# qdrant/quantization

Measured on AMD Instinct MI355X. Metric: scored vectors/sec, 10Mx768 u8 dot, higher is better.
Workload: dtype u8; 1 GPU; 10000000 x 768 store: f32 U[0,1) -> scalar u8 (dot); per step: encode_query + score_all over the shard; quantizer=u8, rows_per_gpu=10000000, dim=768, distance=dot, exchange=scores, gather_group=1, launch=single rank, world_size_seen=1, encode_ahead=False, total_rows=10000000, queries=16

## Files before the change

### quantization_amd/csrc/u8.hip

```cpp
#include <algorithm>
#include <cmath>
#include <cstdlib>
#include <memory>
#include <type_traits>
#include <vector>

#include "common.hpp"
#include "lists.hpp"
#include "multi_reduce.hpp"
#include "topk.hpp"
#include "topk_device.hpp"
#include "rescore.hpp"
#include "u8_internal.hpp"

#pragma clang fp contract(off)

using namespace qamd;

namespace {

constexpr int kBlock = 256;
constexpr int kScanBlock = 512;
constexpr uint64_t kQuantileSample = 100000;

enum Epilogue : int { EPI_POINT = 0, EPI_INTERNAL = 1 };

typedef uint32_t u32x4 __attribute__((ext_vector_type(4)));
typedef float f32x4 __attribute__((ext_vector_type(4)));

__device__ __forceinline__ uint4 ld_nt(const uint4 *p) {
    u32x4 t = __builtin_nontemporal_load(reinterpret_cast<const u32x4 *>(p));
    return make_uint4(t.x, t.y, t.z, t.w);
}
__device__ __forceinline__ float4 ld_nt(const float4 *p) {
    f32x4 t = __builtin_nontemporal_load(reinterpret_cast<const f32x4 *>(p));
    return make_float4(t.x, t.y, t.z, t.w);
}

__device__ __forceinline__ uint32_t dot16(const uint4 &a, const uint4 &b, uint32_t acc) {
    acc = __builtin_amdgcn_udot4(a.x, b.x, acc, false);
    acc = __builtin_amdgcn_udot4(a.y, b.y, acc, false);
    acc = __builtin_amdgcn_udot4(a.z, b.z, acc, false);
    acc = __builtin_amdgcn_udot4(a.w, b.w, acc, false);
    return acc;
}

__device__ __forceinline__ uint32_t sad16(const uint4 &a, const uint4 &b, uint32_t acc) {
    acc = __builtin_amdgcn_sad_u8(a.x, b.x, acc);
    acc = __builtin_amdgcn_sad_u8(a.y, b.y, acc);
    acc = __builtin_amdgcn_sad_u8(a.z, b.z, acc);
    acc = __builtin_amdgcn_sad_u8(a.w, b.w, acc);
    return acc;
}

template <int CTRL> __device__ __forceinline__ uint32_t dpp_add(uint32_t v) {
    return v + (uint32_t)__builtin_amdgcn_update_dpp(0, (int)v, CTRL, 0xF, 0xF, false);
}
template <int G> __device__ __forceinline__ uint32_t group_sum(uint32_t v) {
    static_assert(G == 1 || G == 2 || G == 4 || G == 8 || G == 16, "row group is at most one DPP row");
    if (G >= 2) v = dpp_add<0xB1>(v);
    if (G >= 4) v = dpp_add<0x4E>(v);
    if (G >= 8) v = dpp_add<0x141>(v);
    if (G >= 16) v = dpp_add<0x140>(v);
    return v;
}

__device__ __forceinline__ float epilogue_f(float multiplier, float sf, float q_off, float v_off, float diff, int mode) {
    float ms = multiplier * sf;
    if (mode == EPI_POINT) return (ms + q_off) + v_off;
    return ms + ((q_off + v_off) - diff);
}
__device__ __forceinline__ float epilogue(float multiplier, uint32_t s, float q_off, float v_off,
                                          float diff, int mode) {
    return epilogue_f(multiplier, (float)(int32_t)s, q_off, v_off, diff, mode);
}

__device__ __forceinline__ void dot16_lanes(const uint4 &v, const uint4 &q, uint32_t (&acc)[8]) {
    const uint32_t vd[4] = {v.x, v.y, v.z, v.w};
    const uint32_t qd[4] = {q.x, q.y, q.z, q.w};
#pragma unroll
    for (int j = 0; j < 4; j++) {
        acc[2 * j] = __builtin_amdgcn_udot4(vd[j], qd[j] & 0x0000FFFFu, acc[2 * j], false);
        acc[2 * j + 1] = __builtin_amdgcn_udot4(vd[j], qd[j] & 0xFFFF0000u, acc[2 * j + 1], false);
    }
}
template <int G> __device__ __forceinline__ float avx2_lane_sum(uint32_t (&acc)[8]) {
    float f[8];
#pragma unroll
    for (int k = 0; k < 8; k++) f[k] = (float)(int32_t)group_sum<G>(acc[k]);
    float a0 = f[0] + f[4], a1 = f[1] + f[5], a2 = f[2] + f[6], a3 = f[3] + f[7];
    return (a0 + a2) + (a1 + a3);
}

__device__ __forceinline__ uint32_t f32_to_u8(float v, float alpha, float offset) {
    float x = (v - offset) / alpha;
    x = (x < 0.0f) ? 0.0f : x;
    x = (x > 127.0f) ? 127.0f : x;
    return (x != x) ? 0u : (uint32_t)x;
}

__device__ __forceinline__ bool quant_decided(float y) {
    constexpr float kBand = 3.0517578125e-05f;
    const float fr = __builtin_amdgcn_fractf(y);
    return (__builtin_fabsf(fr - 0.5f) <= 0.5f - kBand) || (__builtin_fabsf(y - 64.0f) >= 64.0f + kBand);
}
__device__ __forceinline__ uint32_t quant_code(float y) {
    return (uint32_t)__builtin_amdgcn_fmed3f(y, 0.0f, 127.0f);
}
__device__ __forceinline__ uint32_t f32x4_to_u8x4_fast(const float4 &f, float alpha, float offset, float r_alpha) {
    const float y0 = (f.x - offset) * r_alpha, y1 = (f.y - offset) * r_alpha, y2 = (f.z - offset) * r_alpha,
                y3 = (f.w - offset) * r_alpha;
    if (quant_decided(y0) && quant_decided(y1) && quant_decided(y2) && quant_decided(y3))
        return quant_code(y0) | (quant_code(y1) << 8) | (quant_code(y2) << 16) | (quant_code(y3) << 24);
    return f32_to_u8(f.x, alpha, offset) | (f32_to_u8(f.y, alpha, offset) << 8) | (f32_to_u8(f.z, alpha, offset) << 16) |
           (f32_to_u8(f.w, alpha, offset) << 24);
}

template <int G, int ITERS, int UNROLL, bool IS_L1, bool EXACT, bool FILTER>
__global__ __launch_bounds__(kScanBlock) void u8_scan_kernel(
    const uint4 *__restrict__ codes, const float *__restrict__ offsets,
    const uint4 *__restrict__ qcodes, const float *__restrict__ q_off_p, float multiplier,
    uint32_t n_rows, uint32_t row_chunks, float *__restrict__ out, TopkFilter filt) {
    constexpr int RW = 64 / G;
    constexpr int TILE = RW * UNROLL;
    const int lane = threadIdx.x & 63;
    const int sub = lane % G;
    const int rslot = lane / G;
    const uint64_t wave = ((uint64_t)blockIdx.x * kScanBlock + threadIdx.x) >> 6;
    const uint64_t base = wave * TILE;
    if (base >= n_rows) return;

    uint4 v[UNROLL][ITERS];
#pragma unroll
    for (int u = 0; u < UNROLL; u++) {
        const uint64_t row = base + u * RW + rslot;
        const uint4 *p = codes + row * row_chunks;
#pragma unroll
        for (int it = 0; it < ITERS; it++) {
            const uint32_t c = sub + it * G;
            if (EXACT) {
                v[u][it] = ld_nt(p + c);
            } else {
                const uint32_t cc = c < row_chunks ? c : row_chunks - 1;
                uint4 t = ld_nt(p + cc);
                const bool in = c < row_chunks;
                v[u][it] = make_uint4(in ? t.x : 0, in ? t.y : 0, in ? t.z : 0, in ? t.w : 0);
            }
        }
    }
    uint4 q[ITERS];
#pragma unroll
    for (int it = 0; it < ITERS; it++) {
        const uint32_t c = sub + it * G;
        if (EXACT) {
            q[it] = qcodes[c];
        } else {
            const uint4 t = qcodes[c < row_chunks ? c : row_chunks - 1];
            const bool in = c < row_chunks;
            q[it] = make_uint4(in ? t.x : 0, in ? t.y : 0, in ? t.z : 0, in ? t.w : 0);
        }
    }
    const float q_off = *q_off_p;
    constexpr int NGROUPS = (UNROLL + G - 1) / G;
    float v_off[NGROUPS];
#pragma unroll
    for (int g = 0; g < NGROUPS; g++)
        v_off[g] = offsets[base + (uint64_t)(g * G + sub) * RW + rslot];
    float mine = 0.0f;
    uint32_t pivot = 0;
    if (FILTER) pivot = *filt.pivot_key;
#pragma unroll
    for (int u = 0; u < UNROLL; u++) {
        uint32_t acc = 0;
#pragma unroll
        for (int it = 0; it < ITERS; it++) acc = IS_L1 ? sad16(v[u][it], q[it], acc) : dot16(v[u][it], q[it], acc);
        acc = group_sum<G>(acc);
        if (sub == (u % G)) mine = epilogue(multiplier, acc, q_off, v_off[u / G], 0.0f, EPI_POINT);
        if ((u % G) == G - 1 || u == UNROLL - 1) {
            constexpr int dummy = 0;
            (void)dummy;
            const int first = (u / G) * G;
            const uint64_t row = base + (uint64_t)(first + sub) * RW + rslot;
            if (sub <= u - first && row < n_rows) {
                if (FILTER) topk_offer(filt, pivot, mine, (uint32_t)row);
                else __builtin_nontemporal_store(mine, out + row);
            }
        }
    }
}

constexpr uint32_t kPackBlockRows = 64;
constexpr uint32_t kPackBlockChunk = kPackBlockRows;

__device__ __forceinline__ uint4 and16(const uint4 &v, uint32_t m) { return make_uint4(v.x & m, v.y & m, v.z & m, v.w & m); }

template <bool FILTER>
__global__ __launch_bounds__(kScanBlock) __attribute__((amdgpu_waves_per_eu(8, 8))) void u8_scan_blocked_kernel(
    const uint4 *__restrict__ image, const float *__restrict__ offsets, const uint4 *__restrict__ qcodes,
    const float *__restrict__ q_off_p, float multiplier, uint32_t n_rows, uint32_t pchunks, uint32_t n_extra,
    uint32_t split, float *__restrict__ out, TopkFilter filt) {
    __shared__ uint32_t partial[kScanBlock];
    const uint32_t lane = threadIdx.x & 63;
    const uint32_t wave = __builtin_amdgcn_readfirstlane(threadIdx.x >> 6);
    const uint32_t part = wave & (split - 1);
    const uint64_t block = (uint64_t)blockIdx.x * ((kScanBlock / 64) / split) + wave / split;
    const uint64_t row = block * kPackBlockRows + lane;
    const bool live = block * kPackBlockRows < n_rows;
    const uint32_t n_rest = pchunks - 7 * n_extra, n_groups = n_extra + (n_rest ? 1 : 0);
    const uint32_t g_begin = live ? n_groups * part / split : 0, g_end = live ? n_groups * (part + 1) / split : 0;
    const uint4 *blk = image + block * pchunks * kPackBlockChunk;
    const uint32_t lane16 = lane * 16;
    auto chunk_ptr = [&](uint32_t c) {
        return reinterpret_cast<const uint4 *>(reinterpret_cast<const char *>(blk + (uint64_t)c * kPackBlockChunk) + lane16);
    };
    const uint32_t gf_end = g_end < n_extra ? g_end : n_extra;
    const bool has_rest = g_end > n_extra;

    uint4 v[7];
    uint32_t acc = 0;
    auto eat = [&](uint32_t g, auto refill) {
        const uint4 *q = qcodes + 7 * g;
        const uint4 qx = qcodes[pchunks + g];
#pragma unroll
        for (int i = 0; i < 7; i++) {
            const uint4 w = v[i];
            acc = dot16(and16(w, 0x7F7F7F7Fu), q[i], acc) + (dot16(and16(w, 0x80808080u), qx, 0) >> (7 - i));
            if (decltype(refill)::value) {
                __builtin_amdgcn_sched_barrier(0);
                v[i] = ld_nt(chunk_ptr(7 * (g + 1) + i));
                __builtin_amdgcn_sched_barrier(0);
            }
        }
    };
    if (g_begin < gf_end) {
#pragma unroll
        for (int i = 0; i < 7; i++) v[i] = ld_nt(chunk_ptr(7 * g_begin + i));
    }
    const float v_off = offsets[row];
    const float q_off = *q_off_p;
    uint32_t pivot = 0;
    if (FILTER) pivot = *filt.pivot_key;
    if (g_begin < gf_end) {
        for (uint32_t g = g_begin; g + 1 < gf_end; g++) eat(g, std::true_type{});
        eat(gf_end - 1, std::false_type{});
    }
    if (has_rest) {
        const uint4 *q = qcodes + 7 * n_extra;
#pragma unroll
        for (int i = 0; i < 7; i++)
            if ((uint32_t)i < n_rest) v[i] = ld_nt(chunk_ptr(7 * n_extra + i));
#pragma unroll
        for (int i = 0; i < 7; i++)
            if ((uint32_t)i < n_rest) acc = dot16(and16(v[i], 0x7F7F7F7Fu), q[i], acc);
    }
    if (split > 1) {
        partial[threadIdx.x] = acc;
        __syncthreads();
        if (part == 0)
            for (uint32_t p = 1; p < split; p++) acc += partial[threadIdx.x + 64 * p];
    }
    if (part == 0 && row < n_rows) {
        const float score = epilogue(multiplier, acc, q_off, v_off, 0.0f, EPI_POINT);
        if (FILTER) topk_offer(filt, pivot, score, (uint32_t)row);
        else __builtin_nontemporal_store(score, out + row);
    }
}

template <int G, int ITERS, int UNROLL, int NQ, bool IS_L1, bool EXACT, bool FILTER>
__global__ __launch_bounds__(kScanBlock) void u8_scan_multi_kernel(
    const uint4 *__restrict__ codes, const float *__restrict__ offsets, const uint8_t *__restrict__ qcodes,
    uint32_t q_pitch, const float *__restrict__ q_offs, uint32_t nq_valid ,
    float multiplier, uint32_t n_rows, uint32_t row_chunks, float *__restrict__ out ,
    uint64_t out_pitch, TopkFilterSlices slices) {
    static_assert(G >= NQ, "one lane of the row group per query");
    constexpr int RW = 64 / G;
    constexpr int TILE = RW * UNROLL;
    constexpr int TPW = NQ;
    const int lane = threadIdx.x & 63;
    const int sub = lane % G, rslot = lane / G;
    const uint64_t wave = ((uint64_t)blockIdx.x * kScanBlock + threadIdx.x) >> 6;
    if (wave * TILE * TPW >= n_rows) return;
    uint4 q[NQ][ITERS];
#pragma unroll
    for (int j = 0; j < NQ; j++) {
        const uint4 *qj = reinterpret_cast<const uint4 *>(qcodes + (size_t)((uint32_t)j < nq_valid ? j : nq_valid - 1) * q_pitch);
#pragma unroll
        for (int it = 0; it < ITERS; it++) {
            const uint32_t c = sub + it * G;
            const bool in = EXACT || c < row_chunks;
            const uint4 t = qj[in ? c : row_chunks - 1];
            q[j][it] = make_uint4(in ? t.x : 0, in ? t.y : 0, in ? t.z : 0, in ? t.w : 0);
        }
    }
    const int my_q = multi_query_of<NQ>(sub);
    const bool owner = sub < NQ && (uint32_t)my_q < nq_valid;
    const float q_off = q_offs[owner ? my_q : 0];
    for (int tile = 0; tile < TPW; tile++) {
        const uint64_t base = (wave * TPW + tile) * TILE;
        if (base >= n_rows) break;
        uint4 v[UNROLL][ITERS];
#pragma unroll
        for (int u = 0; u < UNROLL; u++) {
            const uint4 *p = codes + (base + u * RW + rslot) * row_chunks;
#pragma unroll
            for (int it = 0; it < ITERS; it++) {
                const uint32_t c = sub + it * G;
                const bool in = EXACT || c < row_chunks;
                const uint4 t = ld_nt(p + (in ? c : row_chunks - 1));
                v[u][it] = make_uint4(in ? t.x : 0, in ? t.y : 0, in ? t.z : 0, in ? t.w : 0);
            }
        }
#pragma unroll
        for (int u = 0; u < UNROLL; u++) {
            const uint64_t row = base + (uint64_t)u * RW + rslot;
            const float v_off = offsets[row];
            uint32_t acc[NQ];
#pragma unroll
            for (int j = 0; j < NQ; j++) {
                acc[j] = 0;
#pragma unroll
                for (int it = 0; it < ITERS; it++)
                    acc[j] = IS_L1 ? sad16(v[u][it], q[j][it], acc[j]) : dot16(v[u][it], q[j][it], acc[j]);
            }
            const float mine = epilogue(multiplier, multi_reduce<G, NQ>(acc, sub), q_off, v_off, 0.0f, EPI_POINT);
            if (owner && row < n_rows) {
                if (FILTER) {
                    const TopkFilter f = topk_filter_of(slices, (uint32_t)my_q);
                    topk_offer(f, *f.pivot_key, mine, (uint32_t)row);
                } else {
                    __builtin_nontemporal_store(mine, out + (uint64_t)my_q * out_pitch + row);
                }
            }
        }
    }
}

template <int G, int ITERS, bool IS_L1, bool EXACT>
__device__ __forceinline__ void u8_topk_small_body(const uint4 *__restrict__ codes, const float *__restrict__ offsets,
                                                   const uint4 (&q)[ITERS], float q_off, float multiplier, uint32_t n_rows,
                                                   uint32_t row_chunks, uint32_t rows_per_wg, const SmallTopk &p,
                                                   unsigned long long (*lds)[64]) {
    unsigned long long(*lists)[64] = lds;
    constexpr int RW = 64 / G;
    constexpr int UNROLL = 2;
    const int lane = threadIdx.x & 63, wave = threadIdx.x >> 6;
    const int sub = lane % G, rslot = lane / G;
    unsigned long long *stage = lds[kSmallTopkWaves + wave];
    const uint64_t wg_base = (uint64_t)blockIdx.x * rows_per_wg;
    SmallTopkWave acc_list;
    for (uint32_t tile = wave * UNROLL; tile * RW < rows_per_wg; tile += kSmallTopkWaves * UNROLL) {
        uint4 v[UNROLL][ITERS];
#pragma unroll
        for (int u = 0; u < UNROLL; u++) {
            const uint64_t row = wg_base + (uint64_t)(tile + u) * RW + rslot;
            const uint64_t rc = row < n_rows ? row : (uint64_t)n_rows - 1;
            const uint4 *src = codes + rc * row_chunks;
#pragma unroll
            for (int it = 0; it < ITERS; it++) {
// ... 587 lines not shown
        uint32_t k = (uint32_t)(t - r * row_dwords);
        uint32_t w = rows32[t];
        if (k == 0)
            offsets[r] = __uint_as_float(w);
        else
            codes32[r * (row_dwords - 1) + (k - 1)] = w;
    }
}

__global__ __launch_bounds__(kBlock) void join_rows_kernel(const uint32_t *__restrict__ codes32,
                                                          const float *__restrict__ offsets,
                                                          uint64_t n_rows, uint32_t row_dwords,
                                                          uint32_t *__restrict__ rows32) {
    const uint64_t total = n_rows * row_dwords;
    const uint64_t stride = (uint64_t)gridDim.x * kBlock;
    for (uint64_t t = (uint64_t)blockIdx.x * kBlock + threadIdx.x; t < total; t += stride) {
        uint64_t r = t / row_dwords;
        uint32_t k = (uint32_t)(t - r * row_dwords);
        rows32[t] = k == 0 ? __float_as_uint(offsets[r]) : codes32[r * (row_dwords - 1) + (k - 1)];
    }
}

__global__ __launch_bounds__(kBlock) void u8_pack7_kernel(const uint4 *__restrict__ codes, uint64_t n_rows,
                                                          uint32_t row_chunks, uint32_t pchunks, uint32_t n_extra,
                                                          uint4 *__restrict__ packed, uint32_t *__restrict__ bad) {
    const uint64_t total = n_rows * pchunks, stride = (uint64_t)gridDim.x * kBlock;
    uint32_t high = 0;
    for (uint64_t t = (uint64_t)blockIdx.x * kBlock + threadIdx.x; t < total; t += stride) {
        const uint64_t r = t / pchunks;
        const uint32_t j = (uint32_t)(t - r * pchunks);
        const uint4 *row = codes + r * row_chunks;
        const uint4 a = row[j];
        uint32_t w[4] = {a.x & 0x7F7F7F7Fu, a.y & 0x7F7F7F7Fu, a.z & 0x7F7F7F7Fu, a.w & 0x7F7F7F7Fu};
        high |= a.x | a.y | a.z | a.w;
        if (j < 7 * n_extra) {
            const uint4 x = row[pchunks + j / 7];
            const uint32_t b = j % 7;
            high |= x.x | x.y | x.z | x.w;
            w[0] |= ((x.x >> b) & 0x01010101u) << 7;
            w[1] |= ((x.y >> b) & 0x01010101u) << 7;
            w[2] |= ((x.z >> b) & 0x01010101u) << 7;
            w[3] |= ((x.w >> b) & 0x01010101u) << 7;
        }
        packed[((r / kPackBlockRows) * pchunks + j) * kPackBlockRows + r % kPackBlockRows] = make_uint4(w[0], w[1], w[2], w[3]);
    }
    if (high & 0x80808080u) atomicOr(bad, 1u);
}

__global__ __launch_bounds__(kBlock) void u8_pack7_range_kernel(const uint4 *__restrict__ codes, uint64_t r0, uint64_t n_rows,
                                                                uint32_t row_chunks, uint32_t pchunks, uint32_t n_extra,
                                                                uint4 *__restrict__ packed) {
    const uint64_t total = n_rows * pchunks, stride = (uint64_t)gridDim.x * kBlock;
    for (uint64_t t = (uint64_t)blockIdx.x * kBlock + threadIdx.x; t < total; t += stride) {
        const uint64_t r = r0 + t / pchunks;
        const uint32_t j = (uint32_t)(t % pchunks);
        const uint4 *row = codes + r * row_chunks;
        const uint4 a = row[j];
        uint32_t w[4] = {a.x & 0x7F7F7F7Fu, a.y & 0x7F7F7F7Fu, a.z & 0x7F7F7F7Fu, a.w & 0x7F7F7F7Fu};
        if (j < 7 * n_extra) {
            const uint4 x = row[pchunks + j / 7];
            const uint32_t b = j % 7;
            w[0] |= ((x.x >> b) & 0x01010101u) << 7;
            w[1] |= ((x.y >> b) & 0x01010101u) << 7;
            w[2] |= ((x.z >> b) & 0x01010101u) << 7;
            w[3] |= ((x.w >> b) & 0x01010101u) << 7;
        }
        packed[((r / kPackBlockRows) * pchunks + j) * kPackBlockRows + r % kPackBlockRows] = make_uint4(w[0], w[1], w[2], w[3]);
    }
}

int grid_for(uint64_t work_items, uint64_t per_block, int blocks_per_cu) {
    uint64_t want = (work_items + per_block - 1) / per_block;
    uint64_t cap = (uint64_t)device_info().cu_count * blocks_per_cu;
    if (want < 1) want = 1;
    return (int)(want > cap ? cap : want);
}

float host_multiplier(float alpha, int distance, int invert) {
    float m = distance == QAMD_DOT ? alpha * alpha : distance == QAMD_L1 ? alpha : -2.0f * alpha * alpha;
    return invert ? -m : m;
}

uint64_t actual_dim_of(uint64_t dim) { return dim + (16 - dim % 16) % 16; }

}


namespace {

qamd_status alloc_store(qamd_u8 *h) {
    h->capacity = h->count;
    h->padded_rows = padded_rows_of(h->capacity);
    h->row_chunks = (uint32_t)(h->meta.actual_dim / 16);
    QAMD_TRY(h->codes.alloc_zero_tail(h->padded_rows * h->meta.actual_dim, h->count * h->meta.actual_dim));
    QAMD_TRY(h->offsets.alloc_zero_tail(h->padded_rows * sizeof(float), h->count * sizeof(float)));
    return QAMD_OK;
}

qamd_status build_packed(qamd_u8 *h, hipStream_t s) {
    h->packed.release();
    h->packed_rows.release();
    h->packed_chunks = 0;
    const uint32_t rc = h->row_chunks, n_extra = rc / 8, pchunks = rc - n_extra;
    if (!u8_packed_allowed() || h->count == 0 || rc < 8 || rc > 128 ||
        h->meta.vector_parameters.distance_type == QAMD_L1)
        return QAMD_OK;
    const uint64_t bytes = h->padded_rows * pchunks * 16;
    size_t free_b = 0, total_b = 0;
    if (hipMemGetInfo(&free_b, &total_b) != hipSuccess || free_b < 2 * bytes) {
        (void)hipGetLastError();
        return QAMD_OK;
    }
    DevBuf img, bad;
    const std::string err = last_error();
    if (img.alloc_zero_tail(bytes, h->count / kPackBlockRows * kPackBlockRows * pchunks * 16) != QAMD_OK || bad.alloc(sizeof(uint32_t), true) != QAMD_OK) {
        (void)hipGetLastError();
        last_error() = err;
        return QAMD_OK;
    }
    hipLaunchKernelGGL(u8_pack7_kernel, dim3(grid_for(h->count * pchunks, kBlock, 8)), dim3(kBlock), 0, s,
                       h->codes.as<uint4>(), h->count, rc, pchunks, n_extra, img.as<uint4>(), bad.as<uint32_t>());
    QAMD_HIP(hipGetLastError());
    uint32_t high = 0;
    QAMD_HIP(hipMemcpyAsync(&high, bad.ptr, sizeof(high), hipMemcpyDeviceToHost, s));
    QAMD_HIP(hipStreamSynchronize(s));
    if (high) return QAMD_OK;
    h->packed = std::move(img);
    h->packed_chunks = pchunks;
    return QAMD_OK;
}

template <bool IS_L1> struct ScanLaunch {
    template <int G, int ITERS, int UNROLL>
    static void go(const qamd_u8 *h, const uint4 *qc, const float *qo, float *out, const TopkFilter *filt, hipStream_t s) {
        constexpr int TILE = (64 / G) * UNROLL;
        const uint64_t waves = (h->count + TILE - 1) / TILE;
        const unsigned grid = (unsigned)((waves + kScanBlock / 64 - 1) / (kScanBlock / 64));
        const bool exact = h->row_chunks == (uint32_t)(G * ITERS);
#define QAMD_U8_GO(EX, FI)                                                                                     \
    hipLaunchKernelGGL((u8_scan_kernel<G, ITERS, UNROLL, IS_L1, EX, FI>), dim3(grid), dim3(kScanBlock), 0, s,    \
                       h->codes.as<uint4>(), h->offsets.as<float>(), qc, qo, h->meta.multiplier, (uint32_t)h->count, \
                       h->row_chunks, out, filt ? *filt : TopkFilter{})
        if (filt) {
            if (exact) QAMD_U8_GO(true, true);
            else QAMD_U8_GO(false, true);
        } else {
            if (exact) QAMD_U8_GO(true, false);
            else QAMD_U8_GO(false, false);
        }
#undef QAMD_U8_GO
    }
};

uint32_t blocked_split(uint64_t count) {
    const uint64_t blocks = (count + kPackBlockRows - 1) / kPackBlockRows;
    const uint64_t want = (uint64_t)device_info().cu_count * 16;
    uint32_t split = 1;
    while (split < 8 && blocks * split < want) split *= 2;
    return split;
}

void launch_scan_blocked(const qamd_u8 *h, const uint4 *qc, const float *qo, float *out, const TopkFilter *filt,
                         hipStream_t s) {
    const uint32_t split = blocked_split(h->count), blocks_per_wg = (kScanBlock / 64) / split;
    const uint64_t blocks = (h->count + kPackBlockRows - 1) / kPackBlockRows;
    const unsigned grid = (unsigned)((blocks + blocks_per_wg - 1) / blocks_per_wg);
    h->last_scan_split.store((int)split, std::memory_order_relaxed);
#define QAMD_U8_BLOCKED(FI)                                                                                          \
    hipLaunchKernelGGL((u8_scan_blocked_kernel<FI>), dim3(grid), dim3(kScanBlock), 0, s, h->packed.as<uint4>(),       \
                       h->offsets.as<float>(), qc, qo, h->meta.multiplier, (uint32_t)h->count, h->packed_chunks,      \
                       h->row_chunks - h->packed_chunks, split, out, filt ? *filt : TopkFilter{})
    if (filt) QAMD_U8_BLOCKED(true);
    else QAMD_U8_BLOCKED(false);
#undef QAMD_U8_BLOCKED
}

template <bool IS_L1>
bool launch_scan(const qamd_u8 *h, const uint4 *qc, const float *qo, float *out, const TopkFilter *filt,
                 hipStream_t s) {
    using L = ScanLaunch<IS_L1>;
    const bool packed = !IS_L1 && h->packed_chunks != 0;
    h->last_scan_packed.store(packed ? 1 : 0, std::memory_order_relaxed);
    if (packed) return launch_scan_blocked(h, qc, qo, out, filt, s), true;
    const uint32_t rc = h->row_chunks;
    if (rc == 1) return L::template go<1, 1, 4>(h, qc, qo, out, filt, s), true;
    if (rc == 2) return L::template go<2, 1, 4>(h, qc, qo, out, filt, s), true;
    if (rc <= 4) return L::template go<4, 1, 8>(h, qc, qo, out, filt, s), true;
    if (rc <= 8) return L::template go<8, 1, 8>(h, qc, qo, out, filt, s), true;
    switch ((rc + 15) / 16) {
        case 1: return L::template go<16, 1, 8>(h, qc, qo, out, filt, s), true;
        case 2: return L::template go<16, 2, 4>(h, qc, qo, out, filt, s), true;
        case 3: return L::template go<16, 3, 4>(h, qc, qo, out, filt, s), true;
        case 4: return L::template go<16, 4, 2>(h, qc, qo, out, filt, s), true;
        case 5: return L::template go<16, 5, 2>(h, qc, qo, out, filt, s), true;
        case 6: return L::template go<16, 6, 2>(h, qc, qo, out, filt, s), true;
        case 7: return L::template go<16, 7, 2>(h, qc, qo, out, filt, s), true;
        case 8: return L::template go<16, 8, 2>(h, qc, qo, out, filt, s), true;
        default: break;
    }
    return false;
}

template <bool IS_L1>
void launch_scan_generic(const qamd_u8 *h, const uint4 *qc, const float *qo, float *out, hipStream_t s) {
    uint64_t waves = (h->count + 3) / 4;
    unsigned grid = (unsigned)((waves + kBlock / 64 - 1) / (kBlock / 64));
    hipLaunchKernelGGL((u8_scan_generic_kernel<IS_L1>), dim3(grid), dim3(kBlock), 0, s,
                       h->codes.as<uint4>(), h->offsets.as<float>(), qc, qo, h->meta.multiplier,
                       (uint32_t)h->count, h->row_chunks, out);
}

template <bool IS_L1> struct SmallLaunch {
    template <int G, int ITERS>
    static qamd_status go(const qamd_u8 *h, const uint4 *qc, const float *qo, const FusedQuery *fq, const SmallTopkPlan &pl,
                          const SmallTopk &p, hipStream_t s) {
        const bool exact = h->row_chunks == (uint32_t)(G * ITERS);
        if constexpr (G * ITERS * 16 > (int)kFusedQueryDims + 15 * 16) {
            if (fq) return fail(QAMD_ERR_ARGUMENTS, "fused query does not fit the kernel arguments");
        } else if (fq) {
            QueryByValue qv;
            memcpy(qv.v, fq->values, (size_t)fq->qdim * 4);
            const qamd_vector_parameters &vp = h->meta.vector_parameters;
#define QAMD_U8_SMALL_FUSED(EX)                                                                                        \
    hipLaunchKernelGGL((u8_topk_small_fused_kernel<G, ITERS, IS_L1, EX>), dim3(pl.workgroups), dim3(1024), 0, s,          \
                       h->codes.as<uint4>(), h->offsets.as<float>(), qv, fq->qdim, (uint32_t)h->meta.actual_dim,         \
                       h->meta.alpha, h->meta.offset, vp.distance_type, vp.invert, fq->qbuf, h->meta.multiplier,           \
                       (uint32_t)h->count, h->row_chunks, pl.rows_per_wg, p)
            if (exact) QAMD_U8_SMALL_FUSED(true);
            else QAMD_U8_SMALL_FUSED(false);
#undef QAMD_U8_SMALL_FUSED
            QAMD_HIP(hipGetLastError());
            return QAMD_OK;
        }
#define QAMD_U8_SMALL(EX)                                                                                       \
    hipLaunchKernelGGL((u8_topk_small_kernel<G, ITERS, IS_L1, EX>), dim3(pl.workgroups), dim3(1024), 0, s,       \
                       h->codes.as<uint4>(), h->offsets.as<float>(), qc, qo, h->meta.multiplier, (uint32_t)h->count, \
                       h->row_chunks, pl.rows_per_wg, p)
        if (exact) QAMD_U8_SMALL(true);
        else QAMD_U8_SMALL(false);
#undef QAMD_U8_SMALL
        QAMD_HIP(hipGetLastError());
        return QAMD_OK;
    }
};

int small_group(uint32_t rc) { return rc == 1 ? 1 : rc == 2 ? 2 : rc <= 4 ? 4 : rc <= 8 ? 8 : rc <= 128 ? 16 : 0; }

template <bool IS_L1>
qamd_status launch_small(const qamd_u8 *h, const uint4 *qc, const float *qo, const FusedQuery *fq, const SmallTopkPlan &pl,
                         const SmallTopk &p, hipStream_t s) {
    using L = SmallLaunch<IS_L1>;
    const uint32_t rc = h->row_chunks;
    h->last_scan_packed.store(0, std::memory_order_relaxed);
    if (rc == 1) return L::template go<1, 1>(h, qc, qo, fq, pl, p, s);
    if (rc == 2) return L::template go<2, 1>(h, qc, qo, fq, pl, p, s);
    if (rc <= 4) return L::template go<4, 1>(h, qc, qo, fq, pl, p, s);
    if (rc <= 8) return L::template go<8, 1>(h, qc, qo, fq, pl, p, s);
    switch ((rc + 15) / 16) {
        case 1: return L::template go<16, 1>(h, qc, qo, fq, pl, p, s);
        case 2: return L::template go<16, 2>(h, qc, qo, fq, pl, p, s);
        case 3: return L::template go<16, 3>(h, qc, qo, fq, pl, p, s);
        case 4: return L::template go<16, 4>(h, qc, qo, fq, pl, p, s);
        case 5: return L::template go<16, 5>(h, qc, qo, fq, pl, p, s);
        case 6: return L::template go<16, 6>(h, qc, qo, fq, pl, p, s);
        case 7: return L::template go<16, 7>(h, qc, qo, fq, pl, p, s);
        case 8: return L::template go<16, 8>(h, qc, qo, fq, pl, p, s);
        default: break;
    }
    return fail(QAMD_ERR_ARGUMENTS, "no small top-k kernel for %u chunks", rc);
}

template <bool IS_L1, int G, int ITERS, int UNROLL, int NQ>
void launch_multi_shape(const qamd_u8 *h, const uint8_t *qcodes, uint64_t q_pitch, const float *q_offs, uint32_t nq_valid,
                        float *out, const TopkFilterSlices *slices, hipStream_t s) {
    constexpr int TILE = (64 / G) * UNROLL * NQ;
    const uint64_t waves = (h->count + TILE - 1) / TILE;
    const unsigned grid = (unsigned)((waves + kScanBlock / 64 - 1) / (kScanBlock / 64));
    const bool exact = h->row_chunks == (uint32_t)(G * ITERS);
    h->last_scan_packed.store(0, std::memory_order_relaxed);
#define QAMD_U8_MULTI(EX, FI)                                                                                      \
    hipLaunchKernelGGL((u8_scan_multi_kernel<G, ITERS, UNROLL, NQ, IS_L1, EX, FI>), dim3(grid), dim3(kScanBlock), 0, s, \
                       h->codes.as<uint4>(), h->offsets.as<float>(), qcodes, (uint32_t)q_pitch, q_offs, nq_valid,   \
                       h->meta.multiplier, (uint32_t)h->count, h->row_chunks, out, (uint64_t)h->count,             \
                       slices ? *slices : TopkFilterSlices{})
    if (slices) {
        if (exact) QAMD_U8_MULTI(true, true);
        else QAMD_U8_MULTI(false, true);
    } else {
        if (exact) QAMD_U8_MULTI(true, false);
        else QAMD_U8_MULTI(false, false);
    }
#undef QAMD_U8_MULTI
}

bool lane_order(const qamd_u8 *h) {
    return h->lane_mode == 1 && h->meta.vector_parameters.distance_type != QAMD_L1;
}

uint32_t multi_width(const qamd_u8 *h) {
    const uint32_t rc = h->row_chunks, iters = (rc + 15) / 16;
    const bool l1 = h->meta.vector_parameters.distance_type == QAMD_L1;
    if (rc < 9 || iters > 8 || lane_order(h)) return 0;
    return l1 && iters <= 3 ? 8 : iters <= 6 ? 4 : 2;
}

template <bool IS_L1>
bool launch_multi(const qamd_u8 *h, uint32_t nq_valid, const uint8_t *qcodes, uint64_t q_pitch, const float *q_offs,
                  float *out, const TopkFilterSlices *slices, hipStream_t s) {
    const uint32_t iters = (h->row_chunks + 15) / 16, width = multi_width(h);
    if (nq_valid < 2 || nq_valid > width) return false;
#define QAMD_U8_MULTI_IT(IT, UN)                                                                              \
    case IT:                                                                                                  \
        if constexpr (IS_L1 && IT <= 3) {                                                                     \
            if (nq_valid > 4) {                                                                               \
                launch_multi_shape<IS_L1, 16, IT, UN, 8>(h, qcodes, q_pitch, q_offs, nq_valid, out, slices, s); \
                return true;                                                                                  \
            }                                                                                                 \
        }                                                                                                     \
        if (nq_valid > 2) launch_multi_shape<IS_L1, 16, IT, UN, (IT <= 6 ? 4 : 2)>(h, qcodes, q_pitch, q_offs, nq_valid, out, slices, s); \
        else launch_multi_shape<IS_L1, 16, IT, UN, 2>(h, qcodes, q_pitch, q_offs, nq_valid, out, slices, s);  \
        return true;
    switch (iters) {
        QAMD_U8_MULTI_IT(1, 4) QAMD_U8_MULTI_IT(2, 2) QAMD_U8_MULTI_IT(3, 2) QAMD_U8_MULTI_IT(4, 2)
        QAMD_U8_MULTI_IT(5, 1) QAMD_U8_MULTI_IT(6, 1) QAMD_U8_MULTI_IT(7, 1) QAMD_U8_MULTI_IT(8, 1)
// ... 1036 lines not shown
    return QAMD_OK;
}

qamd_status u8_topk_ptrs(const qamd_u8 *h, const uint8_t *codes_dev, const float *qo, uint32_t k, int largest,
                         uint32_t *out_ids, float *out_scores, qamd_mem out_mem, hipStream_t s, const FusedQuery *fq) {
    const uint4 *qc = reinterpret_cast<const uint4 *>(codes_dev);
    FusedScan scan;
    scan.scan_scores = [&](float *scores, hipStream_t st) { return scan_ptrs(h, qc, qo, scores, st); };
    scan.scan_filter = [&](const TopkFilter &f, hipStream_t st) { return scan_ptrs(h, qc, qo, nullptr, st, &f); };
    scan.score_ids = [&](const uint32_t *ids, uint64_t n_ids, float *out, hipStream_t st) {
        return score_ids_dev(h, qc, qo, 0.0f, EPI_POINT, ids, n_ids, out, st);
    };
    {
        SmallTopkPlan plan;
        if (u8_small_plan(h, k, plan)) {
            const bool is_l1 = h->meta.vector_parameters.distance_type == QAMD_L1;
            return small_topk(plan, k, largest, out_ids, out_scores, out_mem, s,
                              [&](const SmallTopk &p, hipStream_t st) {
                                  return is_l1 ? launch_small<true>(h, qc, qo, fq, plan, p, st)
                                               : launch_small<false>(h, qc, qo, fq, plan, p, st);
                              });
        }
    }
    if (fq) return fail(QAMD_ERR_ARGUMENTS, "a deferred query needs the single-launch path");
    if (!fused_capable(h)) {
        return topk_classic(h->count, k, largest, out_ids, out_scores, out_mem, s,
                            [&](float *scores) { return scan_ptrs(h, qc, qo, scores, s); });
    }
    return fused_topk(h->count, k, largest, out_ids, out_scores, out_mem, s, scan);
}

qamd_status u8_topk_batch_scans(const qamd_u8 *h, const uint8_t *codes_dev, uint64_t pitch, const float *offsets_dev,
                                uint32_t n_queries, uint32_t k, int largest, uint32_t *out_ids, float *out_scores,
                                qamd_mem out_mem, hipStream_t stream) {
    auto qc = [&](uint32_t q) { return reinterpret_cast<const uint4 *>(codes_dev + (uint64_t)q * pitch); };
    BatchScan scan;
    scan.filter_capable = fused_capable(h);
    scan.scan_scores = [&](uint32_t q, float *scores, hipStream_t st) { return scan_ptrs(h, qc(q), offsets_dev + q, scores, st); };
    scan.scan_filter = [&](uint32_t q, const TopkFilter &f, hipStream_t st) {
        return scan_ptrs(h, qc(q), offsets_dev + q, nullptr, st, &f);
    };
    scan.score_ids = [&](uint32_t q, const uint32_t *ids, uint64_t n_ids, float *out, hipStream_t st) {
        return score_ids_dev(h, qc(q), offsets_dev + q, 0.0f, EPI_POINT, ids, n_ids, out, st);
    };
    const bool is_l1 = h->meta.vector_parameters.distance_type == QAMD_L1;
    const uint32_t width = multi_width(h);
    if (width)
        scan.scan_filter_multi = [&, width, is_l1](uint32_t q, uint32_t left, const TopkFilterSlices &sl, hipStream_t st,
                                                   qamd_status &status) -> uint32_t {
            const uint32_t nq = std::min(left, width);
            if (nq < 2) return 0;
            const uint8_t *qcodes = codes_dev + (uint64_t)q * pitch;
            const bool ok = is_l1 ? launch_multi<true>(h, nq, qcodes, pitch, offsets_dev + q, nullptr, &sl, st)
                                  : launch_multi<false>(h, nq, qcodes, pitch, offsets_dev + q, nullptr, &sl, st);
            if (ok && hipGetLastError() != hipSuccess) status = fail(QAMD_ERR_DEVICE, "u8 multi-query filter launch failed");
            return ok ? nq : 0;
        };
    return fused_topk_batch(h->count, n_queries, k, largest, out_ids, out_scores, out_mem, stream, scan);
}

bool u8_host_encode_is_lazy(uint64_t qdim) { return qdim > 0 && actual_dim_of(qdim) <= kFusedQueryDims; }

qamd_status u8_score_lists(const qamd_u8 *h, const uint8_t *codes_dev, uint64_t pitch, const float *offsets_dev,
                           const ListArgs &a, hipStream_t stream) {
    return score_pairs_dev(h, nullptr, nullptr, codes_dev, (uint32_t)pitch, offsets_dev, a.offsets, a.n_lists, nullptr, 0.0f,
                           EPI_POINT, a.ids, a.n_pairs, a.out, stream);
}

uint32_t u8_multi_width(const qamd_u8 *h) { return multi_width(h); }

bool u8_lane_order(const qamd_u8 *h) { return lane_order(h); }

qamd_status u8_score_batch_scans(const qamd_u8 *h, const uint8_t *codes_dev, uint64_t pitch, const float *offsets_dev,
                                 uint32_t n_queries, float *out_dev, hipStream_t stream) {
    const bool is_l1 = h->meta.vector_parameters.distance_type == QAMD_L1;
    const uint32_t width = multi_width(h);
    uint32_t q = 0;
    while (q < n_queries) {
        const uint32_t nq = std::min(width, n_queries - q);
        const uint8_t *qcodes = codes_dev + (uint64_t)q * pitch;
        float *o = out_dev + (uint64_t)q * h->count;
        const bool ok = nq >= 2 && (is_l1 ? launch_multi<true>(h, nq, qcodes, pitch, offsets_dev + q, o, nullptr, stream)
                                          : launch_multi<false>(h, nq, qcodes, pitch, offsets_dev + q, o, nullptr, stream));
        if (ok) {
            q += nq;
        } else {
            QAMD_TRY(scan_ptrs(h, reinterpret_cast<const uint4 *>(qcodes), offsets_dev + q, o, stream));
            q += 1;
        }
    }
    QAMD_HIP(hipGetLastError());
    return QAMD_OK;
}

qamd_status u8_topk_single(const qamd_u8 *h, const uint8_t *codes_dev, const float *offset_dev, uint32_t k,
                           int largest, uint32_t *out_ids, float *out_scores, qamd_mem out_mem, hipStream_t stream) {
    return u8_topk_ptrs(h, codes_dev, offset_dev, k, largest, out_ids, out_scores, out_mem, stream, nullptr);
}

qamd_status u8_score_single(const qamd_u8 *h, const uint8_t *codes_dev, const float *offset_dev, float *out_dev,
                            hipStream_t stream) {
    return scan_ptrs(h, reinterpret_cast<const uint4 *>(codes_dev), offset_dev, out_dev, stream);
}

}

#ifdef QAMD_DEV
extern "C" __attribute__((visibility("default"))) void qamd_dev_u8_ptrs(const qamd_u8 *h, const void **codes,
                                                                        const void **offsets) {
    *codes = h->codes.ptr;
    *offsets = h->offsets.ptr;
}
extern "C" __attribute__((visibility("default"))) const void *qamd_dev_u8_query_ptr(const qamd_u8_query *q) {
    return q->buf.ptr;
}
namespace {
__global__ __launch_bounds__(kBlock) void u8_unblock_kernel(const uint4 *__restrict__ image, uint64_t n_rows,
                                                            uint32_t pchunks, uint4 *__restrict__ rows) {
    const uint64_t total = n_rows * pchunks, stride = (uint64_t)gridDim.x * kBlock;
    for (uint64_t t = (uint64_t)blockIdx.x * kBlock + threadIdx.x; t < total; t += stride) {
        const uint64_t r = t / pchunks;
        const uint32_t j = (uint32_t)(t - r * pchunks);
        rows[t] = image[((r / kPackBlockRows) * pchunks + j) * kPackBlockRows + r % kPackBlockRows];
    }
}
}
extern "C" __attribute__((visibility("default"))) void qamd_dev_u8_packed(const qamd_u8 *h, const void **packed,
                                                                          uint32_t *chunks) {
    *packed = nullptr;
    *chunks = 0;
    if (!h->packed_chunks) return;
    if (!h->packed_rows.ptr) {
        const uint64_t n = h->count * h->packed_chunks;
        if (h->packed_rows.alloc(n * 16, false) != QAMD_OK) return;
        hipLaunchKernelGGL(u8_unblock_kernel, dim3(grid_for(n, kBlock, 8)), dim3(kBlock), 0, nullptr, h->packed.as<uint4>(),
                           h->count, h->packed_chunks, h->packed_rows.as<uint4>());
        if (hipStreamSynchronize(nullptr) != hipSuccess) {
            h->packed_rows.release();
            return;
        }
    }
    *packed = h->packed_rows.ptr;
    *chunks = h->packed_chunks;
}
extern "C" __attribute__((visibility("default"))) void qamd_dev_u8_packed_blocked(const qamd_u8 *h, const void **packed,
                                                                                  uint32_t *chunks, uint32_t *block_rows) {
    *packed = h->packed.ptr;
    *chunks = h->packed_chunks;
    *block_rows = kPackBlockRows;
}
extern "C" __attribute__((visibility("default"))) int qamd_dev_u8_last_scan_split(const qamd_u8 *h) {
    return h->last_scan_split.load(std::memory_order_relaxed);
}
extern "C" __attribute__((visibility("default"))) int qamd_dev_u8_last_scan_packed(const qamd_u8 *h) {
    return h->last_scan_packed.load(std::memory_order_relaxed);
}
#endif

extern "C" qamd_status qamd_u8_topk_rescored(const qamd_u8 *h, const qamd_u8_query *q, const qamd_f32 *orig,
                                              const float *query_f32, uint64_t qdim, qamd_mem query_mem, uint32_t k,
                                              uint32_t candidates, int largest, uint32_t *out_ids, float *out_scores,
                                              qamd_mem out_mem, void *stream) {
    if (!h || !q) return qamd::fail(QAMD_ERR_ARGUMENTS, "null handle or query");
    return qamd::topk_rescored(h->device, h->meta.vector_parameters, orig, query_f32, 1, qdim, query_mem, k, candidates, largest, out_ids,
                               out_scores, out_mem, qamd::as_stream(stream), [&](uint32_t *ids_dev, float *scores_dev) {
                                   return qamd_u8_topk(h, q, candidates, largest, ids_dev, scores_dev, QAMD_MEM_DEVICE, stream);
                               });
}
```

### quantization_amd/csrc/u8_internal.hpp

```cpp
#pragma once
#include <atomic>
#include <mutex>

#include "common.hpp"
#include "lists.hpp"

struct qamd_u8 {
    int device = 0;
    qamd_u8_metadata meta{};
    uint64_t count = 0;
    uint64_t capacity = 0;
    uint64_t padded_rows = 0;
    uint32_t row_chunks = 0;
    int lane_mode = 0;
    qamd::DevBuf codes;
    qamd::DevBuf offsets;
    qamd::DevBuf packed;
    uint32_t packed_chunks = 0;
    mutable std::atomic<int> last_scan_packed{0};
    mutable std::atomic<int> last_scan_split{0};
    mutable qamd::DevBuf packed_rows;
    mutable std::mutex sample_mu;
    mutable qamd::DevBuf sample_codes, sample_offsets;
    mutable uint32_t sample_rows = 0;
};

struct qamd_u8_query {
    int device = 0;
    uint64_t actual_dim = 0;
    qamd::DevBuf buf;
    mutable qamd::ReadyEvent ready;
    mutable std::vector<float> host_f32;
    float alpha = 0.0f, offset = 0.0f;
    int distance = 0, invert = 0;
    mutable std::atomic<bool> deferred{false};
    mutable std::mutex encode_mu;
    bool pooled = false;
    mutable std::atomic<bool> async_used{false};
    ~qamd_u8_query() {
        if (pooled) qamd::query_buf_put(buf, !async_used.load(std::memory_order_relaxed) && ready.complete());
    }
};

namespace qamd {
qamd_status u8_minmax_range(const float *data, qamd_mem mem, uint64_t n_rows, uint64_t dim, hipStream_t s, float *mn,
                            float *mx);
qamd_status u8_quantile_interval(const float *data, qamd_mem mem, uint64_t count, uint64_t dim, float quantile,
                                 hipStream_t s, bool *found, float *mn, float *mx);
}

namespace qamd {
qamd_status u8_encode_queries_device(const qamd_u8 *h, const float *queries_dev, uint64_t n_queries, uint64_t qdim,
                                     uint8_t *codes_dev , uint64_t code_pitch,
                                     float *offsets_dev ,
                                     hipStream_t stream);
bool u8_host_encode_is_lazy(uint64_t qdim);
struct FusedQuery {
    const float *values = nullptr;
    uint32_t qdim = 0;
    uint8_t *qbuf = nullptr;
};
qamd_status u8_topk_ptrs(const qamd_u8 *h, const uint8_t *codes_dev, const float *offset_dev, uint32_t k, int largest,
                         uint32_t *out_ids, float *out_scores, qamd_mem out_mem, hipStream_t stream,
                         const FusedQuery *fq = nullptr);
qamd_status u8_topk_batch_scans(const qamd_u8 *h, const uint8_t *codes_dev, uint64_t pitch, const float *offsets_dev,
                                uint32_t n_queries, uint32_t k, int largest, uint32_t *out_ids, float *out_scores,
                                qamd_mem out_mem, hipStream_t stream);
uint32_t u8_multi_width(const qamd_u8 *h);
bool u8_lane_order(const qamd_u8 *h);
qamd_status u8_score_batch_scans(const qamd_u8 *h, const uint8_t *codes_dev, uint64_t pitch, const float *offsets_dev,
                                 uint32_t n_queries, float *out_dev, hipStream_t stream);
qamd_status u8_score_single(const qamd_u8 *h, const uint8_t *codes_dev, const float *offset_dev, float *out_dev,
                            hipStream_t stream);
qamd_status u8_score_lists(const qamd_u8 *h, const uint8_t *codes_dev, uint64_t pitch, const float *offsets_dev,
                           const ListArgs &a, hipStream_t stream);
qamd_status u8_topk_single(const qamd_u8 *h, const uint8_t *codes_dev, const float *offset_dev, uint32_t k,
                           int largest, uint32_t *out_ids, float *out_scores, qamd_mem out_mem, hipStream_t stream);
}
```

Before: 10.23 billion vectors/s.

## Split blocked u8 scan tail across more waves to balance the last rounds

Splits the blocked scan grid into a head region that keeps the existing per-block wave split and a tail region, sized to a few rounds of CUs, where each 64-row block is split across more waves. The aim is to cut the load imbalance in the final wave of workgroups, so the GPU is not left mostly idle while a few workgroups finish. It adds a per-workgroup branch plus extra partial reductions in the tail, and an env override for the tail size and split.

```diff
diff --git a/quantization_amd/csrc/u8.hip b/quantization_amd/csrc/u8.hip
--- a/quantization_amd/csrc/u8.hip
+++ b/quantization_amd/csrc/u8.hip
@@ -12,6 +12,7 @@
 #include "topk_device.hpp"
 #include "rescore.hpp"
 #include "u8_internal.hpp"
+#include "u8_scan_plan.hpp"
 
 #pragma clang fp contract(off)
 
@@ -198,12 +199,17 @@
 __global__ __launch_bounds__(kScanBlock) __attribute__((amdgpu_waves_per_eu(8, 8))) void u8_scan_blocked_kernel(
     const uint4 *__restrict__ image, const float *__restrict__ offsets, const uint4 *__restrict__ qcodes,
     const float *__restrict__ q_off_p, float multiplier, uint32_t n_rows, uint32_t pchunks, uint32_t n_extra,
-    uint32_t split, float *__restrict__ out, TopkFilter filt) {
+    uint32_t head_split, uint32_t head_wgs, uint32_t tail_split, float *__restrict__ out, TopkFilter filt) {
     __shared__ uint32_t partial[kScanBlock];
     const uint32_t lane = threadIdx.x & 63;
     const uint32_t wave = __builtin_amdgcn_readfirstlane(threadIdx.x >> 6);
+    constexpr uint32_t kWaves = kScanBlock / 64;
+    const bool tail = blockIdx.x >= head_wgs;
+    const uint32_t split = tail ? tail_split : head_split;
     const uint32_t part = wave & (split - 1);
-    const uint64_t block = (uint64_t)blockIdx.x * ((kScanBlock / 64) / split) + wave / split;
+    const uint64_t block = tail ? (uint64_t)head_wgs * (kWaves / head_split) +
+                                      (uint64_t)(blockIdx.x - head_wgs) * (kWaves / tail_split) + wave / tail_split
+                                : (uint64_t)blockIdx.x * (kWaves / head_split) + wave / head_split;
     const uint64_t row = block * kPackBlockRows + lane;
     const bool live = block * kPackBlockRows < n_rows;
     const uint32_t n_rest = pchunks - 7 * n_extra, n_groups = n_extra + (n_rest ? 1 : 0);
@@ -1097,24 +1103,21 @@
     }
 };
 
-uint32_t blocked_split(uint64_t count) {
-    const uint64_t blocks = (count + kPackBlockRows - 1) / kPackBlockRows;
-    const uint64_t want = (uint64_t)device_info().cu_count * 16;
-    uint32_t split = 1;
-    while (split < 8 && blocks * split < want) split *= 2;
-    return split;
-}
+static_assert(kScanPlanBlockRows == kPackBlockRows && kScanPlanWaves == kScanBlock / 64, "u8_scan_plan.hpp");
 
 void launch_scan_blocked(const qamd_u8 *h, const uint4 *qc, const float *qo, float *out, const TopkFilter *filt,
                          hipStream_t s) {
-    const uint32_t split = blocked_split(h->count), blocks_per_wg = (kScanBlock / 64) / split;
-    const uint64_t blocks = (h->count + kPackBlockRows - 1) / kPackBlockRows;
-    const unsigned grid = (unsigned)((blocks + blocks_per_wg - 1) / blocks_per_wg);
-    h->last_scan_split.store((int)split, std::memory_order_relaxed);
+    const uint32_t n_extra = h->row_chunks - h->packed_chunks, n_rest = h->packed_chunks - 7 * n_extra;
+    const U8ScanPlan p = u8_scan_plan(h->count, (uint32_t)device_info().cu_count, n_extra + (n_rest ? 1 : 0),
+                                      u8_scan_tail_parse(dev_env("QAMD_DEV_U8_SCAN_TAIL")));
+    h->last_scan_split.store((int)p.head_split, std::memory_order_relaxed);
+    h->last_scan_tail_blocks.store(p.tail_blocks, std::memory_order_relaxed);
+    h->last_scan_tail_split.store((int)p.tail_split, std::memory_order_relaxed);
 #define QAMD_U8_BLOCKED(FI)                                                                                          \
-    hipLaunchKernelGGL((u8_scan_blocked_kernel<FI>), dim3(grid), dim3(kScanBlock), 0, s, h->packed.as<uint4>(),       \
+    hipLaunchKernelGGL((u8_scan_blocked_kernel<FI>), dim3(p.grid), dim3(kScanBlock), 0, s, h->packed.as<uint4>(),     \
                        h->offsets.as<float>(), qc, qo, h->meta.multiplier, (uint32_t)h->count, h->packed_chunks,      \
-                       h->row_chunks - h->packed_chunks, split, out, filt ? *filt : TopkFilter{})
+                       h->row_chunks - h->packed_chunks, p.head_split, p.head_wgs, p.tail_split, out,                 \
+                       filt ? *filt : TopkFilter{})
     if (filt) QAMD_U8_BLOCKED(true);
     else QAMD_U8_BLOCKED(false);
 #undef QAMD_U8_BLOCKED
@@ -2457,6 +2460,11 @@
 extern "C" __attribute__((visibility("default"))) int qamd_dev_u8_last_scan_split(const qamd_u8 *h) {
     return h->last_scan_split.load(std::memory_order_relaxed);
 }
+extern "C" __attribute__((visibility("default"))) void qamd_dev_u8_last_scan_tail(const qamd_u8 *h, uint64_t *tail_blocks,
+                                                                                  uint32_t *tail_split) {
+    *tail_blocks = h->last_scan_tail_blocks.load(std::memory_order_relaxed);
+    *tail_split = (uint32_t)h->last_scan_tail_split.load(std::memory_order_relaxed);
+}
 extern "C" __attribute__((visibility("default"))) int qamd_dev_u8_last_scan_packed(const qamd_u8 *h) {
     return h->last_scan_packed.load(std::memory_order_relaxed);
 }
diff --git a/quantization_amd/csrc/u8_internal.hpp b/quantization_amd/csrc/u8_internal.hpp
--- a/quantization_amd/csrc/u8_internal.hpp
+++ b/quantization_amd/csrc/u8_internal.hpp
@@ -19,6 +19,8 @@
     uint32_t packed_chunks = 0;
     mutable std::atomic<int> last_scan_packed{0};
     mutable std::atomic<int> last_scan_split{0};
+    mutable std::atomic<uint64_t> last_scan_tail_blocks{0};
+    mutable std::atomic<int> last_scan_tail_split{0};
     mutable qamd::DevBuf packed_rows;
     mutable std::mutex sample_mu;
     mutable qamd::DevBuf sample_codes, sample_offsets;
diff --git a/quantization_amd/csrc/u8_scan_plan.hpp b/quantization_amd/csrc/u8_scan_plan.hpp
--- /dev/null
+++ b/quantization_amd/csrc/u8_scan_plan.hpp
@@ -0,0 +1,77 @@
+#pragma once
+#include <cstdint>
+#include <cstdlib>
+
+namespace qamd {
+
+constexpr uint32_t kScanPlanBlockRows = 64;
+constexpr uint32_t kScanPlanWaves = 8;
+constexpr uint32_t kScanTailRounds = 2;
+constexpr uint32_t kScanTailSplit = 8;
+inline uint32_t u8_scan_default_tail_split(uint32_t groups) {
+    uint32_t split = 1;
+    while (split < kScanTailSplit && split < groups) split *= 2;
+    return split;
+}
+
+struct U8ScanTail {
+    bool set = false;
+    uint64_t blocks = 0;
+    uint32_t split = 1;
+};
+
+inline U8ScanTail u8_scan_tail_parse(const char *text) {
+    U8ScanTail t;
+    if (!text || !*text) return t;
+    char *end = nullptr;
+    const unsigned long long blocks = strtoull(text, &end, 10);
+    if (end == text || *end != ':') return t;
+    const char *s = end + 1;
+    const unsigned long long split = strtoull(s, &end, 10);
+    if (end == s || *end != 0 || split > 8) return t;
+    t.set = true;
+    t.blocks = blocks;
+    t.split = (uint32_t)split;
+    return t;
+}
+
+struct U8ScanPlan {
+    uint32_t head_split = 1, tail_split = 1;
+    uint32_t head_wgs = 0, grid = 0;
+    uint64_t head_blocks = 0, tail_blocks = 0;
+};
+
+inline uint32_t u8_scan_head_split(uint64_t count, uint32_t cu_count) {
+    const uint64_t blocks = (count + kScanPlanBlockRows - 1) / kScanPlanBlockRows;
+    const uint64_t want = (uint64_t)cu_count * 16;
+    uint32_t split = 1;
+    while (split < 8 && blocks * split < want) split *= 2;
+    return split;
+}
+
+inline U8ScanPlan u8_scan_plan(uint64_t count, uint32_t cu_count, uint32_t groups, const U8ScanTail &forced = {}) {
+    U8ScanPlan p;
+    const uint64_t blocks = (count + kScanPlanBlockRows - 1) / kScanPlanBlockRows;
+    p.head_split = u8_scan_head_split(count, cu_count);
+    const uint32_t head_per_wg = kScanPlanWaves / p.head_split;
+    uint64_t want_tail = forced.set ? forced.blocks : (uint64_t)cu_count * 32 * kScanTailRounds;
+    uint32_t tail_split = forced.set ? forced.split : u8_scan_default_tail_split(groups);
+    if (tail_split != 2 && tail_split != 4 && tail_split != 8) tail_split = 1;
+    if (want_tail > blocks) want_tail = blocks;
+    if (tail_split <= p.head_split || want_tail == 0) {
+        p.tail_split = p.head_split;
+        p.head_wgs = (uint32_t)((blocks + head_per_wg - 1) / head_per_wg);
+        p.head_blocks = blocks;
+        p.grid = p.head_wgs;
+        return p;
+    }
+    p.tail_split = tail_split;
+    p.head_wgs = (uint32_t)((blocks - want_tail) / head_per_wg);
+    p.head_blocks = (uint64_t)p.head_wgs * head_per_wg;
+    p.tail_blocks = blocks - p.head_blocks;
+    const uint32_t tail_per_wg = kScanPlanWaves / tail_split;
+    p.grid = p.head_wgs + (uint32_t)((p.tail_blocks + tail_per_wg - 1) / tail_per_wg);
+    return p;
+}
+
+}
```

Result: no change. 10.27 billion vectors/s, median of 6 (+0.4%).
